# kalgeee/Uncertainty-Aware-Multimodal-Emotion-Recognition

Hardware: AMD Instinct MI355X
Metric: samples/sec fwd+bwd at B=4096 (84/256/768-dim) (higher is better)
Workload: dtype bf16; 1 GPU; configs[2]: fusion+DEER forward + MultiTaskDEERLoss + backward (dropout 0.3, gradients materialised in the flat buffer), B=4096/GPU, (B,84)+(B,256)+(B,768) bf16 feature blocks, random-init weights; optimiser step excluded as the metric defines (it maintains the packed weight copies and is timed separately); global_batch=4096, parallelism=single

## Files before the change

uncertainty-aware-multimodal-emotion-recognition_amd/csrc/chain.h:

```cpp
#pragma once
#include "common.h"
#include "nig.h"
#include "options.h"

namespace mmdeer {

constexpr int CHAIN_MAX_SEGS = 12;
constexpr int CHAIN_MAX_VECS = 16;
constexpr int CHAIN_VEC_FLOATS = 4864;

struct ChainSeg {
  const bf16_t* W;
  const float* bias;
  bf16_t* stash;
  const float* gamma;
  const float* beta;
  bf16_t* xln;
  float* out32;
  float* mean;
  float* rstd;
  int N, K, ldw;
  int kin_off, nout_off;
  int dcol_off;
  int ld_stash, nout;
// ... 15 lines not shown
  int residual;
  int res_add, res_dup;
  bf16_t* stash2;
  int stash_split;
};

struct ChainNig {
  int enabled;
  const bf16_t* e2;
  const bf16_t* w3;
  const float* evid;
  const float* targets;
  const float* stats;
  const float* gstats;
  int nblk;
  int nwp;
  bf16_t* dz2;
  float* partial_w;
  float* partial_b;
  float* loss_out;
  int* bin_counts;
  float mask_scale;
  LossCfg cfg;
};

struct ChainNigF {
  int enabled;
  const bf16_t* w3;
  const float* b3;
  int b3_stride;
  float* evid;
  float* nig_out;
  const float* targets;
  float* wstats;
};

struct ChainArgs {
  const bf16_t* X;
  int ldx, K0;
  int B;
  int ts;
  int groups;
  long long group_stride;
  int nseg;
  DropCtx drop;
  const bf16_t* aux_video; const bf16_t* aux_audio; bf16_t* aux_audio_pad;
  int aux_ldv, aux_lda;
  unsigned long long* stamps;
  ChainNig nig;
// ... 38 lines not shown
```

uncertainty-aware-multimodal-emotion-recognition_amd/csrc/chain.hip:

```cpp
#include <type_traits>
#include "gemm_kernel.inc"
#include "chain.h"
#include "options.h"
#include "nig_dev.h"
#include "ln_rows.h"

namespace mmdeer {
namespace {

template <int S>
__device__ __forceinline__ void wr_issue(const void* p) {
  static_assert(S >= 0 && S < 8, "ring slots 0..7");
  if constexpr (S == 0)
    asm volatile("global_load_dwordx4 v[248:251], %0, off\n\tglobal_load_dwordx4 v[252:255], %0, off offset:1024" ::"v"(p)
                 : "memory", "v248", "v249", "v250", "v251", "v252", "v253", "v254", "v255");
  else if constexpr (S == 1)
    asm volatile("global_load_dwordx4 v[240:243], %0, off\n\tglobal_load_dwordx4 v[244:247], %0, off offset:1024" ::"v"(p)
                 : "memory", "v240", "v241", "v242", "v243", "v244", "v245", "v246", "v247");
  else if constexpr (S == 2)
    asm volatile("global_load_dwordx4 v[232:235], %0, off\n\tglobal_load_dwordx4 v[236:239], %0, off offset:1024" ::"v"(p)
                 : "memory", "v232", "v233", "v234", "v235", "v236", "v237", "v238", "v239");
  else if constexpr (S == 3)
    asm volatile("global_load_dwordx4 v[224:227], %0, off\n\tglobal_load_dwordx4 v[228:231], %0, off offset:1024" ::"v"(p)
                 : "memory", "v224", "v225", "v226", "v227", "v228", "v229", "v230", "v231");
// ... 209 lines not shown
  f32x4 ev{0.f, 0.f, 0.f, 0.f};
  float y = 0.f;
  Nig n{0.f, 1.f, 2.f, 1.f};
  Terms t{};
  if (quad_on) {
#pragma unroll
    for (int c = 0; c < 4; ++c) load_chunk16<false>(g.w3, d * 256 + c * 64 + q * 16, w[c]);
    load_chunk16<false>(g.e2, (long long)bc * 192 + d * 64 + q * 16, x);
    ev = *reinterpret_cast<const f32x4*>(g.evid + o * 4);
    y = g.targets[o];
    n = nig_act(ev);
    t = loss_terms(n, y);
  }
  const int stat_n = g.gstats ? (int)g.gstats[3 * NIG_NSTAT] : B;
  NSTAMP(111);
  compute_finals(g.gstats ? g.gstats : g.stats, g.gstats ? 1 : g.nblk, stat_n, g.cfg, F, gs, ftmp, g.gstats ? 0 : g.nwp);
  NSTAMP(112);
  if (blockIdx.x == 0 && tid == 0) write_loss(F, g.loss_out, g.bin_counts);
  if (quad_on) {
    const f32x4 gr = loss_grad(n, t, d, stat_n, g.cfg, F);
    f32x4 dE{gr.x, gr.y * softplus_grad(ev.y), gr.z * softplus_grad(ev.z), gr.w * softplus_grad(ev.w)};
    if (!active) dE = f32x4{0.f, 0.f, 0.f, 0.f};
    float dz[16];
    float* xt = scratch + r * 195 + d * 64 + q * 16;
#pragma unroll
    for (int j = 0; j < 16; ++j) {
      xt[j] = active ? x[j] : 0.f;
      const float v = nig_dx(dE, w[0][j], w[1][j], w[2][j], w[3][j]);
      dz[j] = x[j] > 0.f ? v * g.mask_scale : 0.f;
    }
    if (active) store_chunk16<false>(g.dz2, (long long)b * 192 + d * 64 + q * 16, dz);
// ... 16 lines not shown
    for (int s = 0; s < MS; s += 2) {
      acc0 = fmaf(sde[12 * s], scratch[s * 195 + dd * 64 + j], acc0);
      acc1 = fmaf(sde[12 * s + 12], scratch[(s + 1) * 195 + dd * 64 + j], acc1);
    }
    g.partial_w[(long long)blockIdx.x * 768 + e] = acc0 + acc1;
  }
  if (tid < 12) {
    const float* sde = reinterpret_cast<const float*>(sdE) + tid;
    float bs = 0.f;
    for (int s = 0; s < MS; ++s) bs += sde[12 * s];
    g.partial_b[(long long)blockIdx.x * 12 + tid] = bs;
  }
}

template <int MS>
__device__ __forceinline__ void chain_nig_tail(const ChainNigF& g, const unsigned char* pan, int row0, int B, int tid) {
  const int wave = tid >> 6, lane = tid & 63, q = lane & 3;
  const int qw = wave - (8 - 3 * (MS / 16));
  if (qw < 0) return;
  const int d = qw % 3, blk = qw / 3;
  const int r = 16 * blk + (lane >> 2);
  const int b = row0 + r;
  const bool active = b < B;
  const int bc = active ? b : B - 1;
  float w[4][16], x[16];
#pragma unroll
  for (int c = 0; c < 4; ++c) load_chunk16<false>(g.w3, d * 256 + c * 64 + q * 16, w[c]);
  {
    const unsigned char* prow = pan + d * (MS * 128) + r * 128;
#pragma unroll
    for (int h = 0; h < 2; ++h) {
      const u32x4 raw = *reinterpret_cast<const u32x4*>(prow + (((2 * q + h) ^ (r & 7)) * 16));
      const unsigned dw[4] = {raw.x, raw.y, raw.z, raw.w};
#pragma unroll
// ... 22 lines not shown
  }
  if (g.targets) {
    const float y = g.targets[(long long)bc * 3 + d];
    const Terms t = loss_terms(n, y);
    float* slab = g.wstats + ((long long)((row0 >> 4) + blk) * 3 + d) * NIG_NSTAT;
    float v[NIG_NSTAT];
    v[0] = writer ? t.logprob : 0.f; v[1] = writer ? t.reg : 0.f; v[2] = writer ? t.kla : 0.f; v[3] = writer ? t.klb : 0.f; v[4] = writer ? t.u : 0.f;
#pragma unroll
    for (int k = 0; k < 10; ++k) {
      const bool in = writer && t.bin == k;
      v[5 + k] = in ? t.conf : 0.f; v[15 + k] = in ? t.aerr : 0.f; v[25 + k] = in ? 1.f : 0.f;
    }
#pragma unroll
    for (int i = 0; i < NIG_NSTAT; ++i) {
      const float sm = wave_sum(v[i]);
      if (lane == 0) slab[i] = sm;
    }
  }
}

template <int D, int VECF, int TS>
__device__ __forceinline__ void chain_body(const ChainKArgs& a) {
  constexpr int MS = 16 * TS, LOG_MS = TS == 1 ? 4 : 5, FLY = 2 * D;
  constexpr int G = D == 8 ? 4 : D;
  constexpr int PAN = TS == 1 ? MS * 1536 : MS * 1024;
  constexpr int AUXB = TS == 1 ? MS * 768 : 0;
  constexpr int AUX = 2 * PAN, RED = AUX + AUXB, VEC = RED + 32768, TAB = VEC + VECF * 4;
  constexpr int SEG_BYTES = (int)sizeof(ChainRecK);
  constexpr int VEC0 = CHAIN_MAX_SEGS * SEG_BYTES;
  constexpr int TAB_BYTES = VEC0 + CHAIN_MAX_VECS * (int)sizeof(ChainVecK);
  static_assert(TAB_BYTES % 16 == 0 && TAB_BYTES / 16 <= 512, "one 16-byte chunk of the tables per thread");
  static_assert(TAB + TAB_BYTES <= 160 * 1024, "LDS budget");
  __shared__ __attribute__((aligned(1024))) unsigned char lds[TAB + TAB_BYTES];
// ... 487 lines not shown
      }
      stamp(131 + 4 * si);
      if (has_ln) {
        asm volatile("s_waitcnt lgkmcnt(0)" ::: "memory");
        __builtin_amdgcn_s_barrier();
      }
      unsigned char* t = pin; pin = pout; pout = t;
      rows_in = rows_out;
    }
#pragma unroll
    for (int k = 0; k < SEG_DW; ++k) rs[k] = rn[k];
#pragma unroll
    for (int k = 0; k < 8; ++k) rl[k] = rln[k];
    stamp(5 + 3 * si);
  }
  if (a.nigf.enabled) chain_nig_tail<MS>(a.nigf, pin, row0, B, tid);
  asm volatile("s_waitcnt vmcnt(0)" ::: "memory");
}

__global__ __launch_bounds__(512) __attribute__((amdgpu_num_vgpr(112))) void chain_kernel_s16(const ChainKArgs a) {
  chain_body<4, CHAIN_VEC_FLOATS, 1>(a);
}
__global__ __launch_bounds__(512) __attribute__((amdgpu_num_vgpr(96))) void chain_kernel_s16_d8(const ChainKArgs a) {
  chain_body<8, CHAIN_VEC_FLOATS, 1>(a);
}
__global__ __launch_bounds__(512) __attribute__((amdgpu_num_vgpr(120))) void chain_kernel_s32(const ChainKArgs a) {
  chain_body<2, CHAIN_VEC_FLOATS, 2>(a);
}
__global__ __launch_bounds__(512) __attribute__((amdgpu_num_vgpr(120))) void chain_kernel_s16_d2(const ChainKArgs a) {
  chain_body<2, CHAIN_VEC_FLOATS, 1>(a);
}
// ... 114 lines not shown
    MMDEER_CHECK(ts == 1 && !a.nig.enabled && a.groups == 1, "chain: the second input panel needs 16-sample workgroups and a single-group input");
    MMDEER_CHECK(a.aux_audio && a.aux_audio_pad && ((uintptr_t)a.aux_video % 16) == 0 && a.aux_ldv % 8 == 0 && ((uintptr_t)a.aux_audio % 4) == 0 &&
                     a.aux_lda % 2 == 0 && a.aux_lda <= 128 && ((uintptr_t)a.aux_audio_pad % 16) == 0,
                 "chain: second input panel: pointers / alignment");
  }
  ChainKArgs k{};
  k.aux_video = a.aux_video; k.aux_audio = a.aux_audio; k.aux_audio_pad = a.aux_audio_pad; k.aux_ldv = a.aux_ldv; k.aux_lda = a.aux_lda;
  k.X = a.X; k.ldx = a.ldx; k.K0 = a.K0; k.B = a.B; k.groups = a.groups; k.group_stride = a.group_stride; k.drop = a.drop;
  k.stamps = a.stamps;
  k.nig = a.nig;
  k.nigf = a.nigf;
  if (a.nigf.enabled) {
    const ChainSeg& last = a.seg[a.nseg - 1];
    MMDEER_CHECK(!a.nig.enabled && last.end_layer && last.nout == 192 && !last.gamma && !last.lnb_gamma && last.fold_groups == 0,
                 "chain: the NIG tail needs a plain 192-wide last layer");
    MMDEER_CHECK(a.nigf.w3 && a.nigf.b3 && a.nigf.evid && a.nigf.nig_out && (!a.nigf.targets || a.nigf.wstats) &&
                     ((uintptr_t)a.nigf.w3 % 16) == 0 && ((uintptr_t)a.nigf.evid % 16) == 0,
                 "chain: NIG tail: NULL argument / alignment");
  }
  int vec = 0, nend = 0, nvec = 0;
  int blocks_in = a.groups * ts, width_in = a.K0, layer_first_seg = 0;
  bool layer_has_group1 = false, width_in_dup = false;
  auto add_vec = [&](const float* src, int n) { ChainVecK& v = k.vec[nvec++]; v.src = src; v.off = vec; v.n4 = n / 4; vec += n; return v.off; };
  for (int i = 0; i < a.nseg; ++i) {
    const ChainSeg& s = a.seg[i];
    MMDEER_CHECK(s.W && ((uintptr_t)s.W % 16) == 0, "chain: segment %d weights (fragment-major image) must be 16-byte aligned", i);
    MMDEER_CHECK(s.N > 0 && s.N % 64 == 0 && s.K > 0 && s.K % 64 == 0 && (s.N % 128 == 0 || s.K % 128 == 0),
                 "chain: segment %d has unsupported N = %d, K = %d", i, s.N, s.K);
    MMDEER_CHECK(!s.in_aux || a.aux_video, "chain: segment %d reads a second input panel the chain does not have", i);
    MMDEER_CHECK(s.kin_off >= 0 && s.kin_off % 64 == 0 && s.kin_off + s.K <= (s.in_aux ? 384 : width_in), "chain: segment %d reads columns [%d, %d) of a %d-wide panel", i,
                 s.kin_off, s.kin_off + s.K, s.in_aux ? 384 : width_in);
    MMDEER_CHECK(s.row_group == 0 || (s.row_group == 1 && s.fold_groups == 0 && blocks_in == ts), "chain: segment %d row group", i);
// ... 97 lines not shown
```

uncertainty-aware-multimodal-emotion-recognition_amd/csrc/common.h:

```cpp
#pragma once
#include <hip/hip_runtime.h>
#include <stdint.h>

#include <initializer_list>

namespace mmdeer {

typedef unsigned short bf16_t;
typedef __bf16 bf16x8 __attribute__((ext_vector_type(8)));
typedef float f32x4 __attribute__((ext_vector_type(4)));

__device__ __forceinline__ void store_wt4(float* p, float v) {
  asm volatile("global_store_dword %0, %1, off sc0 sc1" ::"v"(p), "v"(v) : "memory");
}
template <typename V2>
__device__ __forceinline__ void store_wt8(void* p, V2 v) {
  static_assert(sizeof(V2) == 8, "store_wt8 writes 8 bytes");
  asm volatile("global_store_dwordx2 %0, %1, off sc0 sc1" ::"v"(p), "v"(v) : "memory");
}
template <typename V4>
__device__ __forceinline__ void store_wt16(void* p, V4 v) {
  static_assert(sizeof(V4) == 16, "store_wt16 writes 16 bytes");
  asm volatile("global_store_dwordx4 %0, %1, off sc0 sc1\n\ts_nop 1" ::"v"(p), "v"(v) : "memory");
}

enum { DT_BF16 = 0, DT_F32 = 1 };

__device__ __forceinline__ float bf2f(bf16_t h) { return __uint_as_float(((unsigned)h) << 16); }
__device__ __forceinline__ bf16_t f2bf(float f) { return __builtin_bit_cast(unsigned short, (__bf16)f); }
typedef float f32x2_t __attribute__((ext_vector_type(2)));
typedef __bf16 bf16x2_t __attribute__((ext_vector_type(2)));
__device__ __forceinline__ unsigned pack_bf2(float lo, float hi) {
  return __builtin_bit_cast(unsigned, __builtin_convertvector(f32x2_t{lo, hi}, bf16x2_t));
}

template <typename T> struct Elem;
template <> struct Elem<float> {
  static constexpr int EPC = 4;
// ... 139 lines not shown
```

uncertainty-aware-multimodal-emotion-recognition_amd/csrc/gemm_tt256.hip:

```cpp
#include "gemm_kernel.inc"
#include "rowops.h"

#include <type_traits>

namespace mmdeer {
namespace {

__device__ __forceinline__ void gload16_sc1(f32x4& dst, const void* p) {
  asm volatile("global_load_dwordx4 %0, %1, off sc1" : "=v"(dst) : "v"(p) : "memory");
}
__device__ __forceinline__ void gload4_sc1(float& dst, const void* p) {
  asm volatile("global_load_dword %0, %1, off sc1" : "=v"(dst) : "v"(p) : "memory");
}

constexpr int fold_round(int want, int all) {
  int r = 1;
  while (2 * r <= want && 2 * r <= all) r *= 2;
  return r;
}

__device__ __forceinline__ void fold_tail(int tb, unsigned char* lds) {
  const __attribute__((address_space(4))) GemmFold& F =
      *(const __attribute__((address_space(4))) GemmFold*)((karg_ptr)__builtin_amdgcn_kernarg_segment_ptr() + __builtin_offsetof(GemmGroup, fold));
  const int half = threadIdx.x >> 8, b = 2 * tb + half;
  int sg = 0;
#pragma unroll
  for (int i = 1; i < GEMM_FOLD_SEGMENTS; ++i)
    if (i < F.nseg && b >= F.bstart[i]) sg = i;
// ... 344 lines not shown
```

uncertainty-aware-multimodal-emotion-recognition_amd/csrc/layout.inc:

```
X(W, ACT,  wpack,    MMDEER_FLAT_ELEMS, 0)
X(W, ACT,  wtpack,   MMDEER_FLAT_ELEMS, 0)
X(W, F32,  vpack,    MMDEER_FLAT_ELEMS, 0)
X(W, BF16, wa_pad,   INTER * AUD_PAD, 0)
X(W, BF16, wqkv_hm,  3 * FUS * FUS, 0)
X(W, F32,  wscratch, ADAM_NPART, 0)
X(W, BF16, wfpack,   MMDEER_FLAT_ELEMS, 1)
X(W, BF16, wtfpack,  MMDEER_FLAT_ELEMS, 1)
X(W, BF16, wa_frag,  INTER * AUD_PAD, 1)
X(S, BF16, audio_pad, Bz * AUD_PAD, 0)
X(S, ACT, avin, 2 * Bz * INTER, 0) X(S, ACT, avv, 2 * Bz * INTER, 0) X(S, ACT, cat, Bz * 2 * INTER, 0) X(S, ACT, y_a2, Bz * INTER, 0)
X(S, ACT, av, Bz * INTER, 0) X(S, ACT, xtok, 2 * Bz * FUS, 0) X(S, ACT, qkv, 2 * Bz * 3 * FUS, 0) X(S, ACT, obar, Bz * FUS, 0)
X(S, ACT, pool, Bz * FUS, 0) X(S, ACT, y_t3, Bz * FUS, 0) X(S, ACT, tri, Bz * FUS, 0) X(S, ACT, y_o1, Bz * FUS, 0) X(S, ACT, fused, Bz * FUS, 0)
X(S, ACT, h1, Bz * HID, 0) X(S, ACT, h2, Bz * HID, 0) X(S, ACT, e1, Bz * 3 * EV1, 0) X(S, ACT, e2, Bz * 3 * EV2, 0)
X(S, F32, probs, Bz * 8 * 4, 0) X(S, F32, evid, Bz * 12, 0)
X(S, F32, stats, 4 * nblk * 3 * NIG_NSTAT, 0)
X(S, F32, mean_a2, Bz, 0) X(S, F32, rstd_a2, Bz, 0) X(S, F32, mean_t3, Bz, 0) X(S, F32, rstd_t3, Bz, 0) X(S, F32, mean_o1, Bz, 0) X(S, F32, rstd_o1, Bz, 0)
X(S, ACT, dz2, Bz * 3 * EV2, 0) X(S, ACT, de1, Bz * 3 * EV1, 0) X(S, ACT, dh2, Bz * HID, 0) X(S, ACT, dh1, Bz * HID, 0)
X(S, ACT, dfused, Bz * FUS, 0) X(S, ACT, dz_o1, Bz * FUS, 0) X(S, ACT, dtri, Bz * FUS, 0) X(S, ACT, dz_t3, Bz * FUS, 0)
X(S, ACT, dpool, Bz * FUS, 0) X(S, ACT, dobar, Bz * FUS, 0) X(S, ACT, dqkv, 2 * Bz * 3 * FUS, 0) X(S, ACT, dxtok, 2 * Bz * FUS, 0)
X(S, ACT, dav, Bz * INTER, 0) X(S, ACT, dz_a2, Bz * INTER, 0) X(S, ACT, dcats, 2 * Bz * INTER, 0) X(S, ACT, davv, 2 * Bz * INTER, 0)
X(S, ACT, davin, 2 * Bz * INTER, 0)
X(S, F32, part_ln_o1, np * 2 * FUS, 0) X(S, F32, part_ln_t3, np * 2 * FUS, 0) X(S, F32, part_ln_a2, np * 2 * INTER, 0)
X(S, F32, part_w3, nhead * 3 * 256, 0) X(S, F32, part_b3, nhead * 3 * 4, 0)
X(S, F32, slab, SPLITK_MAX * MMDEER_FLAT_ELEMS, 0)
```

uncertainty-aware-multimodal-emotion-recognition_amd/csrc/nig.h:

```cpp
#pragma once
#include "common.h"

struct mmdeer_loss_cfg;

namespace mmdeer {

constexpr int NIG_NSTAT = 35;
constexpr int NIG_GLOBAL_STATS = 3 * NIG_NSTAT + 1;
constexpr int NIG_LOSS_OUT = 20;

struct LossCfg {
  float reg_w, kl_w, ece_w, cross_w;
  float task_w[3];
};
LossCfg loss_cfg(const mmdeer_loss_cfg& c);

constexpr int NIG_ROWS = 64;
inline int nig_nblocks(int B) { return B > 0 ? (B + NIG_ROWS - 1) / NIG_ROWS : 1; }

int launch_nig_fwd(const void* e2, const void* w3, const float* b3, int b3_stride, float* evid, float* nig_out,
                   const float* targets, float* stats, int B, int act_f32, hipStream_t s);

int launch_nig_bwd(const void* e2, const void* w3, const float* evid, const float* targets, const float* stats,
                   const float* gstats, const float* gmu, const float* gnu, const float* galpha, const float* gbeta,
                   float* devid, void* dz2, float* partial_w, float* partial_b, float* loss_out, int* bin_counts,
                   int B, int act_f32, float mask_scale, const LossCfg& cfg, int nwp, hipStream_t s);

int launch_nig_stats_sum(const float* stats, int B, float* out, int nwp, hipStream_t s);

int launch_nig_loss_stats(const float* gamma, const float* nu, const float* alpha, const float* beta,
                          const float* targets, float* stats, int B, hipStream_t s);
int launch_nig_loss_grad(const float* gamma, const float* nu, const float* alpha, const float* beta,
                         const float* targets, const float* stats, float* dgamma, float* dnu, float* dalpha,
                         float* dbeta, float* loss_out, int* bin_counts, int B, const LossCfg& cfg, hipStream_t s);

int deer_v1_nblocks(long long n);
int launch_deer_loss_v1(const float* mu, const float* nu, const float* alpha, const float* beta, const float* targets, long long n,
                        float ew, float kw, float* loss_out, float* dmu, float* dnu, float* dalpha, float* dbeta, float* partial,
                        hipStream_t s);
int launch_unc_reg_loss(const float* alpha, const float* beta, int B, int D, float dw, float sw, float* loss_out, float* dalpha,
                        float* dbeta, hipStream_t s);
// ... 11 lines not shown
```

uncertainty-aware-multimodal-emotion-recognition_amd/csrc/nig.hip:

```cpp
#include "nig.h"
#include "stamps.h"

namespace mmdeer {
namespace {
#ifdef MMDEER_STAMPS
__device__ unsigned long long g_nig_stamps[16];
#define GSTAMP(slot) MMDEER_STAMP((unsigned long long*)g_nig_stamps, slot, blockIdx.x == 0 && blockIdx.y == 0 && threadIdx.x == 0)
#endif
}
}
#include "nig_dev.h"

namespace mmdeer {
namespace {



template <bool F32>
__global__ __launch_bounds__(256) void nig_fwd_kernel(const void* e2, const void* w3, const float* b3, int b3_stride,
                                                      float* evid, float* nig_out, const float* targets, float* stats, int B) {
  const int d = blockIdx.y, tid = threadIdx.x, q = tid & 3;
  const int b = blockIdx.x * NIG_ROWS + (tid >> 2);
  const bool active = b < B;
  const int bc = active ? b : B - 1;
// ... 21 lines not shown
    nig_out[o] = n.mu; nig_out[plane + o] = n.nu; nig_out[2 * plane + o] = n.alpha; nig_out[3 * plane + o] = n.beta;
    nig_out[4 * plane + o] = alea; nig_out[5 * plane + o] = epis; nig_out[6 * plane + o] = alea + epis;
  }
  if (targets) {
    const float y = targets[(long long)bc * 3 + d];
    const Terms t = loss_terms(n, y);
    block_stats(t, writer, stats + ((long long)blockIdx.x * 3 + d) * NIG_NSTAT);
  }
}

template <bool F32>
__global__ __launch_bounds__(256) void nig_bwd_kernel(const void* e2, const void* w3, const float* evid, const float* targets,
                                                      const float* stats, const float* gstats, const float* gmu,
                                                      const float* gnu, const float* galpha, const float* gbeta, float* devid, void* dz2,
                                                      float* partial_w, float* partial_b, float* loss_out,
                                                      int* bin_counts, int B, float mask_scale, LossCfg cfg, int nwp) {
  __shared__ float gs[3][NIG_NSTAT];
  __shared__ float ftmp[NIG_FINALS_TMP];
  __shared__ f32x4 sdE[NIG_ROWS];
  __shared__ Finals F;
  __shared__ float xt[NIG_ROWS][65];
  const int d = blockIdx.y, tid = threadIdx.x, q = tid & 3, s = tid >> 2;
  const int nblk = gridDim.x;
  const int b = blockIdx.x * NIG_ROWS + s;
  const bool active = b < B;
  const int bc = active ? b : B - 1;
  const long long o = (long long)bc * 3 + d;
  GSTAMP(0);
  float w[4][16];
#pragma unroll
  for (int c = 0; c < 4; ++c) load_chunk16<F32>(w3, d * 256 + c * 64 + q * 16, w[c]);
  float x[16];
  load_chunk16<F32>(e2, (long long)bc * 192 + d * 64 + q * 16, x);
  const f32x4 ev = *reinterpret_cast<const f32x4*>(evid + o * 4);
  const bool loss_mode = targets != nullptr;
  f32x4 g{0.f, 0.f, 0.f, 0.f};
  if (loss_mode) {
    const float y = targets[o];
    GSTAMP(1);
    const int stat_n = gstats ? (int)gstats[3 * NIG_NSTAT] : B;
    compute_finals(gstats ? gstats : stats, gstats ? 1 : nblk, stat_n, cfg, F, gs, ftmp, gstats ? 0 : nwp);
    GSTAMP(2);
    if (blockIdx.x == 0 && blockIdx.y == 0 && tid == 0) write_loss(F, loss_out, bin_counts);
    const Nig n = nig_act(ev);
    const Terms t = loss_terms(n, y);
    g = loss_grad(n, t, d, stat_n, cfg, F);
    GSTAMP(3);
  } else {
    if (gmu) g.x = gmu[o];
    if (gnu) g.y = gnu[o];
    if (galpha) g.z = galpha[o];
    if (gbeta) g.w = gbeta[o];
  }
  f32x4 dE{g.x, g.y * softplus_grad(ev.y), g.z * softplus_grad(ev.z), g.w * softplus_grad(ev.w)};
  if (!active) dE = f32x4{0.f, 0.f, 0.f, 0.f};
  if (active && q == 0 && devid) *reinterpret_cast<f32x4*>(devid + o * 4) = dE;
// ... 249 lines not shown
  } else if (i == 3 * NIG_NSTAT) {
    out[i] = (float)B;
  }
}

int launch_nig_stats_sum(const float* stats, int B, float* out, int nwp, hipStream_t s) {
  MMDEER_CHECK(B > 0, "nig statistics need a non-empty batch");
  hipLaunchKernelGGL(nig_stats_sum_kernel, dim3(1), dim3(128), 0, s, stats, nig_nblocks(B), B, out, nwp);
  MMDEER_HIP(hipGetLastError());
  return 0;
}

int launch_nig_bwd(const void* e2, const void* w3, const float* evid, const float* targets, const float* stats,
                   const float* gstats, const float* gmu, const float* gnu, const float* galpha, const float* gbeta,
                   float* devid, void* dz2, float* partial_w, float* partial_b, float* loss_out, int* bin_counts,
                   int B, int act_f32, float mask_scale, const LossCfg& cfg, int nwp, hipStream_t s) {
  MMDEER_CHECK(B > 0, "nig backward needs a non-empty batch");
  dim3 grid(nig_nblocks(B), 3);
  if (act_f32)
    hipLaunchKernelGGL(nig_bwd_kernel<true>, grid, dim3(256), 0, s, e2, w3, evid, targets, stats, gstats, gmu, gnu, galpha, gbeta,
                       devid, dz2, partial_w, partial_b, loss_out, bin_counts, B, mask_scale, cfg, nwp);
  else
    hipLaunchKernelGGL(nig_bwd_kernel<false>, grid, dim3(256), 0, s, e2, w3, evid, targets, stats, gstats, gmu, gnu, galpha, gbeta,
                       devid, dz2, partial_w, partial_b, loss_out, bin_counts, B, mask_scale, cfg, nwp);
  MMDEER_HIP(hipGetLastError());
  return 0;
}

int launch_nig_loss_stats(const float* gamma, const float* nu, const float* alpha, const float* beta,
                          const float* targets, float* stats, int B, hipStream_t s) {
  MMDEER_CHECK(B > 0, "nig loss needs a non-empty batch");
  hipLaunchKernelGGL(nig_loss_stats_kernel, dim3((B + 255) / 256, 3), dim3(256), 0, s, gamma, nu, alpha, beta, targets, stats, B);
  MMDEER_HIP(hipGetLastError());
  return 0;
}

int launch_nig_loss_grad(const float* gamma, const float* nu, const float* alpha, const float* beta,
                         const float* targets, const float* stats, float* dgamma, float* dnu, float* dalpha,
                         float* dbeta, float* loss_out, int* bin_counts, int B, const LossCfg& cfg, hipStream_t s) {
// ... 52 lines not shown
```

uncertainty-aware-multimodal-emotion-recognition_amd/csrc/nig_dev.h:

```cpp
#pragma once
#include "nig.h"
#include "elem.h"

#ifndef GSTAMP
#define GSTAMP(slot) do {} while (0)
#endif

namespace mmdeer {
namespace {

typedef unsigned nig_u32x4 __attribute__((ext_vector_type(4)));

__device__ const float kEceEdges[11] = {0.0f, 0x1.99999ap-4f, 0x1.99999ap-3f, 0x1.333334p-2f, 0x1.99999ap-2f, 0x1p-1f,
                                        0x1.333334p-1f, 0x1.666666p-1f, 0x1.99999ap-1f, 0x1.ccccccp-1f, 1.0f};
constexpr float kEps = 1e-8f;
constexpr float kTwoPiEps = 6.28318530717958647692f;



struct Nig { float mu, nu, alpha, beta; };

__device__ __forceinline__ Nig nig_act(const f32x4& ev) {
#pragma clang fp contract(off)
  Nig n;
// ... 59 lines not shown
    if (lane == 0) sm[wave][i] = s;
  }
  __syncthreads();
  if (threadIdx.x < NIG_NSTAT)
    slab[threadIdx.x] = (sm[0][threadIdx.x] + sm[1][threadIdx.x]) + (sm[2][threadIdx.x] + sm[3][threadIdx.x]);
}

struct Finals {
  float sign[3][10];
  float dcross[3];
  float out[NIG_LOSS_OUT];
  int counts[3][10];
};

constexpr int NIG_FINALS_TMP = 3 * NIG_NSTAT + 30 + 3 + 3;
__device__ __forceinline__ void compute_finals(const float* stats, int nblk, int B, const LossCfg& cfg, Finals& F,
                                               float (*gs)[NIG_NSTAT], float* tmp, int nwp = 0) {
  constexpr int NV = 3 * NIG_NSTAT;
  float* const upper = tmp; float* const ece_c = tmp + NV; float* const dim_total = ece_c + 30; float* const ubar_s = dim_total + 3;
  {
    const int i = threadIdx.x & 127, h = threadIdx.x >> 7;
    float acc = 0.f;
    if (i < NV) {
      const int per = (nblk + 1) >> 1, p0 = h * per, p1 = (p0 + per < nblk) ? p0 + per : nblk;
      if (nwp == 0) {
        for (int q = p0; q < p1; q += 16) {
          float v[16];
#pragma unroll
          for (int u = 0; u < 16; ++u) {
            const int p = q + u < p1 ? q + u : p1 - 1;
            v[u] = stats[(long long)p * NV + i];
          }
#pragma unroll
          for (int u = 0; u < 16; ++u) v[u] = q + u < p1 ? v[u] : 0.f;
          acc += ((v[0] + v[1]) + (v[2] + v[3])) + ((v[4] + v[5]) + (v[6] + v[7])) +
                 (((v[8] + v[9]) + (v[10] + v[11])) + ((v[12] + v[13]) + (v[14] + v[15])));
        }
      } else {
        for (int q = p0; q < p1; q += 16) {
          float w[16][4];
#pragma unroll
          for (int u = 0; u < 16; ++u)
#pragma unroll
            for (int z = 0; z < 4; ++z) {
              const int p = q + u < p1 ? q + u : p1 - 1, wp = 4 * p + z;
              w[u][z] = stats[(long long)(wp < nwp ? wp : nwp - 1) * NV + i];
            }
          float v[16];
#pragma unroll
          for (int u = 0; u < 16; ++u) {
            const int p = q + u < p1 ? q + u : p1 - 1;
#pragma unroll
            for (int z = 0; z < 4; ++z) w[u][z] = 4 * p + z < nwp ? w[u][z] : 0.f;
            v[u] = q + u < p1 ? (w[u][0] + w[u][1]) + (w[u][2] + w[u][3]) : 0.f;
          }
          acc += ((v[0] + v[1]) + (v[2] + v[3])) + ((v[4] + v[5]) + (v[6] + v[7])) +
                 (((v[8] + v[9]) + (v[10] + v[11])) + ((v[12] + v[13]) + (v[14] + v[15])));
        }
      }
      if (h == 1) upper[i] = acc;
    }
    __syncthreads();
    if (h == 0 && i < NV) gs[i / NIG_NSTAT][i % NIG_NSTAT] = acc + upper[i];
  }
  GSTAMP(8);
  __syncthreads();
  GSTAMP(9);
  const float N = (float)B;
  if (threadIdx.x < 30) {
    const int d = threadIdx.x / 10, k = threadIdx.x - d * 10;
    const float cnt = gs[d][25 + k];
    F.counts[d][k] = (int)cnt;
    float sg = 0.f, c = 0.f;
    if (cnt > 0.f) {
      const float diff = gs[d][5 + k] / cnt - (1.0f - gs[d][15 + k] / cnt);
      c = (cnt / N) * fabsf(diff);
      sg = diff > 0.f ? 1.f : (diff < 0.f ? -1.f : 0.f);
    }
// ... 120 lines not shown
```

uncertainty-aware-multimodal-emotion-recognition_amd/csrc/stackc.hip:

```cpp
#include <cstring>

#include "../../include/mmdeer.h"
#include "../../include/mmdeer_routes.h"
#include "attention.h"
#include "common.h"
#include "gemm.h"
#include "nig.h"
#include "optim.h"
#include "options.h"
#include "chain.h"
#include "rowops.h"

namespace mmdeer {
namespace {

constexpr int TRACE_MAX = 32;
struct Trace { void** ev = nullptr; int max = 0, n = 0; const char* label[TRACE_MAX]; };
thread_local Trace g_trace;
int trace_mark(const char* label, hipStream_t s) {
  Trace& t = g_trace;
  if (!t.ev || t.n >= t.max || t.n >= TRACE_MAX) return 0;
  if (hipEventRecord((hipEvent_t)t.ev[t.n], s) != hipSuccess) { set_error("trace: hipEventRecord failed"); return -1; }
  t.label[t.n++] = label;
  return 0;
// ... 22 lines not shown
constexpr int P_AVP_W = MMDEER_P_TRIMODAL_AUDIOVISUAL_PROJECTION_WEIGHT, P_AVP_B = MMDEER_P_TRIMODAL_AUDIOVISUAL_PROJECTION_BIAS;
constexpr int P_TXT_W = MMDEER_P_TRIMODAL_TEXT_PROJECTION_WEIGHT, P_TXT_B = MMDEER_P_TRIMODAL_TEXT_PROJECTION_BIAS;
constexpr int P_TIN_W = MMDEER_P_TRIMODAL_MODALITY_ATTENTION_IN_PROJ_WEIGHT, P_TIN_B = MMDEER_P_TRIMODAL_MODALITY_ATTENTION_IN_PROJ_BIAS;
constexpr int P_TOUT_W = MMDEER_P_TRIMODAL_MODALITY_ATTENTION_OUT_PROJ_WEIGHT, P_TOUT_B = MMDEER_P_TRIMODAL_MODALITY_ATTENTION_OUT_PROJ_BIAS;
constexpr int P_TFF_W = MMDEER_P_TRIMODAL_FINAL_0_WEIGHT, P_TFF_B = MMDEER_P_TRIMODAL_FINAL_0_BIAS;
constexpr int P_TFF_G = MMDEER_P_TRIMODAL_FINAL_3_WEIGHT, P_TFF_BT = MMDEER_P_TRIMODAL_FINAL_3_BIAS;
constexpr int P_OP_W = MMDEER_P_OUTP0_WEIGHT, P_OP_B = MMDEER_P_OUTP0_BIAS, P_OP_G = MMDEER_P_OUTP3_WEIGHT, P_OP_BT = MMDEER_P_OUTP3_BIAS;
constexpr int P_FP0_W = MMDEER_P_FP0_WEIGHT, P_FP0_B = MMDEER_P_FP0_BIAS, P_FP1_W = MMDEER_P_FP3_WEIGHT, P_FP1_B = MMDEER_P_FP3_BIAS;
constexpr int P_EV0_W = MMDEER_P_HEAD0_EV0_WEIGHT, P_EV0_B = MMDEER_P_HEAD0_EV0_BIAS;
constexpr int P_EV1_W = MMDEER_P_HEAD0_EV3_WEIGHT, P_EV1_B = MMDEER_P_HEAD0_EV3_BIAS;
constexpr int P_EV2_W = MMDEER_P_HEAD0_EV6_WEIGHT, P_EV2_B = MMDEER_P_HEAD0_EV6_BIAS;

constexpr int AUD = MMDEER_AUDIO_DIM, VID = MMDEER_VIDEO_DIM, TXT = MMDEER_TEXT_DIM, INTER = MMDEER_INTER_DIM;
constexpr int FUS = MMDEER_FUSION_DIM, HID = MMDEER_HIDDEN_DIM, EV1 = 128, EV2 = 64;
constexpr int SPLITK_MAX = 8;
constexpr int AUD_PAD = 128;

struct Layout {
  using ACT = char; using BF16 = char; using F32 = float;
#define X(buf, kind, name, elems, bf16_only) kind* name;
#include "layout.inc"
#undef X
  size_t wbytes;
  size_t bytes;
};

inline size_t align_up(size_t x, size_t a = 256) { return (x + a - 1) / a * a; }

Layout make_layout(void* base, void* wbase, int B, int f32) {
  Layout L{};
// ... 565 lines not shown
  }
  if (plan.chains) {
    ChainArgs c = X.chain(n.tout.in, n.tout.K, 1, 0);
    X.fwd_seg(c, n.tout);
    X.fwd_seg(c, n.tff);
    X.fwd_seg(c, n.op);
    X.fwd_seg(c, n.fp0);
    X.fwd_seg(c, n.fp1);
    X.fwd_seg(c, n.ev0);
    X.fwd_seg(c, n.ev1);
    if (plan.nig_tail) {
      ChainNigF& g = c.nigf;
      g.enabled = 1;
      g.w3 = reinterpret_cast<const bf16_t*>(X.W(P_EV2_W)); g.b3 = X.V(P_EV2_B); g.b3_stride = 64;
      g.evid = L.evid; g.nig_out = a->nig_out; g.targets = a->targets; g.wstats = L.stats;
    }
#ifdef MMDEER_STAMPS
    c.stamps = reinterpret_cast<unsigned long long*>(L.slab);
#endif
    TRY(launch_chain(c, s));
    MARK(plan.nig_tail ? "chain F9-F18 (trimodal fusion tail + head + NIG)" : "chain F9-F17 (trimodal fusion tail + head)");
  } else {
    TRY(X.run1(X.fwd(n.tout)));
    TRY(X.run1(X.fwd(n.tff)));
    if (lnf) {
      TRY(X.fwd_ln(n.op, n.tff));
      TRY(X.fwd_ln(n.fp0, n.op));
    } else {
      TRY(X.ln_fwd(n.tff));
      TRY(X.run1(X.fwd(n.op)));
// ... 59 lines not shown
      TRY(X.run(dwg));
      MARK("weight gradients (all problems, one launch)");
      for (int i = 0; i < dwg.nprob; ++i) Exec::add_slab_segments(rt, dwg.p[i]);
    }
    if (!fold_in) {
      rt.bump = bump;
      TRY(launch_reduce_partials(rt, s));
      MARK("reduce_partials (fold)");
    }
    for (int b = first_bucket; b <= last_bucket; ++b)
      if (a->bucket_events[b]) MMDEER_HIP(hipEventRecord((hipEvent_t)a->bucket_events[b], s));
    return 0;
  };

  if (phase != 2) {
  if (!plan.nigfold)
    TRY(launch_nig_bwd(L.e2, X.W(P_EV2_W), L.evid, a->targets, L.stats, a->targets ? a->global_stats : nullptr, a->g_mu, a->g_nu, a->g_alpha, a->g_beta, nullptr,
                       L.dz2, L.part_w3, L.part_b3, a->loss_out, a->bin_counts, B, f32, X.mask_scale, cfg, plan.nwp, s));
  if (!plan.nigfold) MARK("nig_bwd (head's last layer backward + loss gradient)");
  if (plan.bchain) {
    ChainArgs c = X.chain(n.ev1.dout, n.ev1.heads * n.ev1.N, 1, 0);
    X.dx_seg(c, n.ev1);
    X.dx_seg(c, n.ev0);
    X.dx_seg(c, n.fp1);
    X.dx_seg(c, n.fp0, &n.op);
    X.dx_seg(c, n.op, &n.tff);
    X.dx_seg(c, n.tff);
    X.dx_seg(c, n.tout);
    if (plan.nigfold) {
      ChainNig& g = c.nig;
      g.enabled = 1;
      g.e2 = reinterpret_cast<const bf16_t*>(L.e2); g.w3 = reinterpret_cast<const bf16_t*>(X.W(P_EV2_W)); g.evid = L.evid;
      g.targets = a->targets; g.stats = L.stats; g.gstats = a->global_stats; g.nblk = nblk; g.nwp = plan.nwp;
      g.dz2 = reinterpret_cast<bf16_t*>(L.dz2); g.partial_w = L.part_w3; g.partial_b = L.part_b3;
      g.loss_out = a->loss_out; g.bin_counts = a->bin_counts; g.mask_scale = X.mask_scale; g.cfg = cfg;
    }
#ifdef MMDEER_STAMPS
    c.stamps = reinterpret_cast<unsigned long long*>(L.davin);
#endif
    TRY(launch_chain(c, s));
    MARK(plan.nigfold ? "chain B1-B10 (head backward + loss gradient + head / trimodal dX)" : "chain B2-B10 (head / trimodal dX)");
  } else {
    TRY(X.run1(X.dx(n.ev1)));
    TRY(X.run1(X.dx(n.ev0)));
    TRY(X.run1(X.dx(n.fp1)));
    TRY(X.run1(X.dx(n.fp0)));
  }
  if (a->g_fused) TRY(launch_add_f32(L.dfused, f32, a->g_fused, (long long)B * FUS, s));
// ... 135 lines not shown
```

uncertainty-aware-multimodal-emotion-recognition_amd/model.py:

```python
from __future__ import annotations

import ctypes as C
import math
from dataclasses import dataclass
from typing import Dict, Optional, Tuple

import torch
import torch.nn as nn

from . import _lib, synth
from .spec import DEFAULT_DIMS, DIM_NAMES, Dims, gate_param_table, param_offsets, param_table

LOSS_KEYS = ("total_loss", "nll_loss", "reg_loss", "kl_loss", "ece_loss")


@dataclass
class ModelConfig:

    audio_dim: int = 84
    video_dim: int = 256
    text_dim: int = 768
    encoder_dim: int = 256
    fusion_dim: int = 512
    emotion_dims: int = 3
# ... 187 lines not shown
        self.fusion.load_state_dict(fusion_sd)
        self.head.load_state_dict(head_sd)

    def load_numpy_state(self, state) -> None:
        sd = {k: torch.as_tensor(v) for k, v in state.items()}
        own = self.state_dict()
        for k in own:
            if k in sd:
                own[k].copy_(sd[k])

    def _workspace(self, B: int, dev: torch.device) -> torch.Tensor:
        key = (B, self.compute_f32, dev.index if dev.index is not None else 0)
        ws = self._st.workspaces.get(key)
        if ws is None:
            nbytes = _lib.load().mmdeer_workspace_bytes(B, self.compute_f32)
            ws = torch.empty(nbytes, dtype=torch.uint8, device=dev)
            self._st.workspaces[key] = ws
        return ws

    def _weights(self, dev: torch.device) -> torch.Tensor:
        key = (self.compute_f32, dev.index if dev.index is not None else 0)
        wb = self._st.weights.get(key)
        if wb is None:
            wb = torch.empty(_lib.load().mmdeer_weights_bytes(self.compute_f32), dtype=torch.uint8, device=dev)
            self._st.weights[key] = wb
            self._st.packed_key = None
        return wb

    def _param_key(self, wb: torch.Tensor):
        return (wb.data_ptr(), self._st.param_gen) + tuple((p.data_ptr(), p._version) for p in self._live)

# ... 392 lines not shown
```

Baseline: 15.67 million samples/s.

## Fold NIG loss statistics in the last forward chain workgroup via atomic ticket

The forward chain's NIG tail now takes an atomic ticket per workgroup, and the last workgroup to finish sums all per-wave statistic partials into a small global fold buffer. The backward loss-gradient code then reads this pre-folded block as if it were global stats, instead of every backward workgroup re-reducing all the per-wave partials. This removes redundant reductions from the backward critical path. In exchange it adds a grid-wide atomic, a wait on outstanding stores and cache-bypassing loads at the end of the forward pass, and requires the workspace to be zero-initialised so the counter starts at zero.

```diff
diff --git a/uncertainty-aware-multimodal-emotion-recognition_amd/csrc/chain.h b/uncertainty-aware-multimodal-emotion-recognition_amd/csrc/chain.h
--- a/uncertainty-aware-multimodal-emotion-recognition_amd/csrc/chain.h
+++ b/uncertainty-aware-multimodal-emotion-recognition_amd/csrc/chain.h
@@ -53,7 +53,6 @@
   const float* stats;
   const float* gstats;
   int nblk;
-  int nwp;
   bf16_t* dz2;
   float* partial_w;
   float* partial_b;
@@ -72,6 +71,8 @@
   float* nig_out;
   const float* targets;
   float* wstats;
+  float* fold;
+  unsigned* cnt;
 };
 
 struct ChainArgs {
diff --git a/uncertainty-aware-multimodal-emotion-recognition_amd/csrc/chain.hip b/uncertainty-aware-multimodal-emotion-recognition_amd/csrc/chain.hip
--- a/uncertainty-aware-multimodal-emotion-recognition_amd/csrc/chain.hip
+++ b/uncertainty-aware-multimodal-emotion-recognition_amd/csrc/chain.hip
@@ -247,7 +247,7 @@
   }
   const int stat_n = g.gstats ? (int)g.gstats[3 * NIG_NSTAT] : B;
   NSTAMP(111);
-  compute_finals(g.gstats ? g.gstats : g.stats, g.gstats ? 1 : g.nblk, stat_n, g.cfg, F, gs, ftmp, g.gstats ? 0 : g.nwp);
+  compute_finals(g.gstats ? g.gstats : g.stats, g.gstats ? 1 : g.nblk, stat_n, g.cfg, F, gs, ftmp);
   NSTAMP(112);
   if (blockIdx.x == 0 && tid == 0) write_loss(F, g.loss_out, g.bin_counts);
   if (quad_on) {
@@ -294,10 +294,8 @@
 }
 
 template <int MS>
-__device__ __forceinline__ void chain_nig_tail(const ChainNigF& g, const unsigned char* pan, int row0, int B, int tid) {
-  const int wave = tid >> 6, lane = tid & 63, q = lane & 3;
-  const int qw = wave - (8 - 3 * (MS / 16));
-  if (qw < 0) return;
+__device__ __forceinline__ void chain_nig_rows(const ChainNigF& g, const unsigned char* pan, int row0, int B, int qw, int lane) {
+  const int q = lane & 3;
   const int d = qw % 3, blk = qw / 3;
   const int r = 16 * blk + (lane >> 2);
   const int b = row0 + r;
@@ -350,9 +348,28 @@
 #pragma unroll
     for (int i = 0; i < NIG_NSTAT; ++i) {
       const float sm = wave_sum(v[i]);
-      if (lane == 0) slab[i] = sm;
-    }
-  }
+      if (lane == 0) store_wt4(slab + i, sm);
+    }
+  }
+}
+
+template <int MS>
+__device__ __forceinline__ void chain_nig_tail(const ChainNigF& g, const unsigned char* pan, float* scratch, int row0, int B, int tid) {
+  const int qw = (tid >> 6) - (8 - 3 * (MS / 16));
+  if (qw >= 0) chain_nig_rows<MS>(g, pan, row0, B, qw, tid & 63);
+  if (!g.targets) return;
+  asm volatile("s_waitcnt vmcnt(0)" ::: "memory");
+  __builtin_amdgcn_s_barrier();
+  volatile unsigned* ticket = reinterpret_cast<volatile unsigned*>(scratch);
+  if (tid == 0) *ticket = __hip_atomic_fetch_add(g.cnt, 1u, __ATOMIC_RELAXED, __HIP_MEMORY_SCOPE_AGENT);
+  __syncthreads();
+  if (*ticket != gridDim.x - 1) return;
+  __builtin_amdgcn_fence(__ATOMIC_ACQUIRE, "wavefront");
+  const int nwp = (B + 15) >> 4;
+  const float sum = sum_stat_partials<true, true>(g.wstats, (nwp + 3) >> 2, nwp, scratch + 16);
+  if (tid < 3 * NIG_NSTAT) g.fold[tid] = sum;
+  else if (tid == 3 * NIG_NSTAT) g.fold[tid] = (float)B;
+  if (tid == 0) __hip_atomic_store(g.cnt, 0u, __ATOMIC_RELAXED, __HIP_MEMORY_SCOPE_AGENT);
 }
 
 template <int D, int VECF, int TS>
@@ -870,7 +887,7 @@
     for (int k = 0; k < 8; ++k) rl[k] = rln[k];
     stamp(5 + 3 * si);
   }
-  if (a.nigf.enabled) chain_nig_tail<MS>(a.nigf, pin, row0, B, tid);
+  if (a.nigf.enabled) chain_nig_tail<MS>(a.nigf, pin, reinterpret_cast<float*>(pout), row0, B, tid);
   asm volatile("s_waitcnt vmcnt(0)" ::: "memory");
 }
 
@@ -1015,8 +1032,8 @@
     const ChainSeg& last = a.seg[a.nseg - 1];
     MMDEER_CHECK(!a.nig.enabled && last.end_layer && last.nout == 192 && !last.gamma && !last.lnb_gamma && last.fold_groups == 0,
                  "chain: the NIG tail needs a plain 192-wide last layer");
-    MMDEER_CHECK(a.nigf.w3 && a.nigf.b3 && a.nigf.evid && a.nigf.nig_out && (!a.nigf.targets || a.nigf.wstats) &&
-                     ((uintptr_t)a.nigf.w3 % 16) == 0 && ((uintptr_t)a.nigf.evid % 16) == 0,
+    MMDEER_CHECK(a.nigf.w3 && a.nigf.b3 && a.nigf.evid && a.nigf.nig_out && (!a.nigf.targets || (a.nigf.wstats && a.nigf.fold && a.nigf.cnt)) &&
+                     ((uintptr_t)a.nigf.w3 % 16) == 0 && ((uintptr_t)a.nigf.evid % 16) == 0 && ((uintptr_t)a.nigf.cnt % 4) == 0,
                  "chain: NIG tail: NULL argument / alignment");
   }
   int vec = 0, nend = 0, nvec = 0;
diff --git a/uncertainty-aware-multimodal-emotion-recognition_amd/csrc/common.h b/uncertainty-aware-multimodal-emotion-recognition_amd/csrc/common.h
--- a/uncertainty-aware-multimodal-emotion-recognition_amd/csrc/common.h
+++ b/uncertainty-aware-multimodal-emotion-recognition_amd/csrc/common.h
@@ -22,6 +22,12 @@
 __device__ __forceinline__ void store_wt16(void* p, V4 v) {
   static_assert(sizeof(V4) == 16, "store_wt16 writes 16 bytes");
   asm volatile("global_store_dwordx4 %0, %1, off sc0 sc1\n\ts_nop 1" ::"v"(p), "v"(v) : "memory");
+}
+__device__ __forceinline__ void gload16_sc1(f32x4& dst, const void* p) {
+  asm volatile("global_load_dwordx4 %0, %1, off sc1" : "=v"(dst) : "v"(p) : "memory");
+}
+__device__ __forceinline__ void gload4_sc1(float& dst, const void* p) {
+  asm volatile("global_load_dword %0, %1, off sc1" : "=v"(dst) : "v"(p) : "memory");
 }
 
 enum { DT_BF16 = 0, DT_F32 = 1 };
diff --git a/uncertainty-aware-multimodal-emotion-recognition_amd/csrc/gemm_tt256.hip b/uncertainty-aware-multimodal-emotion-recognition_amd/csrc/gemm_tt256.hip
--- a/uncertainty-aware-multimodal-emotion-recognition_amd/csrc/gemm_tt256.hip
+++ b/uncertainty-aware-multimodal-emotion-recognition_amd/csrc/gemm_tt256.hip
@@ -5,13 +5,6 @@
 
 namespace mmdeer {
 namespace {
-
-__device__ __forceinline__ void gload16_sc1(f32x4& dst, const void* p) {
-  asm volatile("global_load_dwordx4 %0, %1, off sc1" : "=v"(dst) : "v"(p) : "memory");
-}
-__device__ __forceinline__ void gload4_sc1(float& dst, const void* p) {
-  asm volatile("global_load_dword %0, %1, off sc1" : "=v"(dst) : "v"(p) : "memory");
-}
 
 constexpr int fold_round(int want, int all) {
   int r = 1;
diff --git a/uncertainty-aware-multimodal-emotion-recognition_amd/csrc/layout.inc b/uncertainty-aware-multimodal-emotion-recognition_amd/csrc/layout.inc
--- a/uncertainty-aware-multimodal-emotion-recognition_amd/csrc/layout.inc
+++ b/uncertainty-aware-multimodal-emotion-recognition_amd/csrc/layout.inc
@@ -22,4 +22,6 @@
 X(S, ACT, davin, 2 * Bz * INTER, 0)
 X(S, F32, part_ln_o1, np * 2 * FUS, 0) X(S, F32, part_ln_t3, np * 2 * FUS, 0) X(S, F32, part_ln_a2, np * 2 * INTER, 0)
 X(S, F32, part_w3, nhead * 3 * 256, 0) X(S, F32, part_b3, nhead * 3 * 4, 0)
-X(S, F32, slab, SPLITK_MAX * MMDEER_FLAT_ELEMS, 0)
+X(S, F32, slab, SPLITK_MAX * MMDEER_FLAT_ELEMS - NIG_FOLD_ELEMS, 0)
+X(S, F32, nig_fold, 128, 0)
+X(S, F32, nig_cnt, 64, 0)
diff --git a/uncertainty-aware-multimodal-emotion-recognition_amd/csrc/nig.h b/uncertainty-aware-multimodal-emotion-recognition_amd/csrc/nig.h
--- a/uncertainty-aware-multimodal-emotion-recognition_amd/csrc/nig.h
+++ b/uncertainty-aware-multimodal-emotion-recognition_amd/csrc/nig.h
@@ -24,7 +24,7 @@
 int launch_nig_bwd(const void* e2, const void* w3, const float* evid, const float* targets, const float* stats,
                    const float* gstats, const float* gmu, const float* gnu, const float* galpha, const float* gbeta,
                    float* devid, void* dz2, float* partial_w, float* partial_b, float* loss_out, int* bin_counts,
-                   int B, int act_f32, float mask_scale, const LossCfg& cfg, int nwp, hipStream_t s);
+                   int B, int act_f32, float mask_scale, const LossCfg& cfg, hipStream_t s);
 
 int launch_nig_stats_sum(const float* stats, int B, float* out, int nwp, hipStream_t s);
 
diff --git a/uncertainty-aware-multimodal-emotion-recognition_amd/csrc/nig.hip b/uncertainty-aware-multimodal-emotion-recognition_amd/csrc/nig.hip
--- a/uncertainty-aware-multimodal-emotion-recognition_amd/csrc/nig.hip
+++ b/uncertainty-aware-multimodal-emotion-recognition_amd/csrc/nig.hip
@@ -59,7 +59,7 @@
                                                       const float* stats, const float* gstats, const float* gmu,
                                                       const float* gnu, const float* galpha, const float* gbeta, float* devid, void* dz2,
                                                       float* partial_w, float* partial_b, float* loss_out,
-                                                      int* bin_counts, int B, float mask_scale, LossCfg cfg, int nwp) {
+                                                      int* bin_counts, int B, float mask_scale, LossCfg cfg) {
   __shared__ float gs[3][NIG_NSTAT];
   __shared__ float ftmp[NIG_FINALS_TMP];
   __shared__ f32x4 sdE[NIG_ROWS];
@@ -84,7 +84,7 @@
     const float y = targets[o];
     GSTAMP(1);
     const int stat_n = gstats ? (int)gstats[3 * NIG_NSTAT] : B;
-    compute_finals(gstats ? gstats : stats, gstats ? 1 : nblk, stat_n, cfg, F, gs, ftmp, gstats ? 0 : nwp);
+    compute_finals(gstats ? gstats : stats, gstats ? 1 : nblk, stat_n, cfg, F, gs, ftmp);
     GSTAMP(2);
     if (blockIdx.x == 0 && blockIdx.y == 0 && tid == 0) write_loss(F, loss_out, bin_counts);
     const Nig n = nig_act(ev);
@@ -364,15 +364,15 @@
 int launch_nig_bwd(const void* e2, const void* w3, const float* evid, const float* targets, const float* stats,
                    const float* gstats, const float* gmu, const float* gnu, const float* galpha, const float* gbeta,
                    float* devid, void* dz2, float* partial_w, float* partial_b, float* loss_out, int* bin_counts,
-                   int B, int act_f32, float mask_scale, const LossCfg& cfg, int nwp, hipStream_t s) {
+                   int B, int act_f32, float mask_scale, const LossCfg& cfg, hipStream_t s) {
   MMDEER_CHECK(B > 0, "nig backward needs a non-empty batch");
   dim3 grid(nig_nblocks(B), 3);
   if (act_f32)
     hipLaunchKernelGGL(nig_bwd_kernel<true>, grid, dim3(256), 0, s, e2, w3, evid, targets, stats, gstats, gmu, gnu, galpha, gbeta,
-                       devid, dz2, partial_w, partial_b, loss_out, bin_counts, B, mask_scale, cfg, nwp);
+                       devid, dz2, partial_w, partial_b, loss_out, bin_counts, B, mask_scale, cfg);
   else
     hipLaunchKernelGGL(nig_bwd_kernel<false>, grid, dim3(256), 0, s, e2, w3, evid, targets, stats, gstats, gmu, gnu, galpha, gbeta,
-                       devid, dz2, partial_w, partial_b, loss_out, bin_counts, B, mask_scale, cfg, nwp);
+                       devid, dz2, partial_w, partial_b, loss_out, bin_counts, B, mask_scale, cfg);
   MMDEER_HIP(hipGetLastError());
   return 0;
 }
diff --git a/uncertainty-aware-multimodal-emotion-recognition_amd/csrc/nig_dev.h b/uncertainty-aware-multimodal-emotion-recognition_amd/csrc/nig_dev.h
--- a/uncertainty-aware-multimodal-emotion-recognition_amd/csrc/nig_dev.h
+++ b/uncertainty-aware-multimodal-emotion-recognition_amd/csrc/nig_dev.h
@@ -97,22 +97,33 @@
 };
 
 constexpr int NIG_FINALS_TMP = 3 * NIG_NSTAT + 30 + 3 + 3;
-__device__ __forceinline__ void compute_finals(const float* stats, int nblk, int B, const LossCfg& cfg, Finals& F,
-                                               float (*gs)[NIG_NSTAT], float* tmp, int nwp = 0) {
+
+template <bool WAVE, bool SC1>
+__device__ __forceinline__ float sum_stat_partials(const float* stats, int nblk, int nwp, float* upper) {
   constexpr int NV = 3 * NIG_NSTAT;
-  float* const upper = tmp; float* const ece_c = tmp + NV; float* const dim_total = ece_c + 30; float* const ubar_s = dim_total + 3;
+  auto ld = [](const float* p) __attribute__((always_inline)) {
+    float v;
+    if constexpr (SC1) gload4_sc1(v, p);
+    else v = *p;
+    return v;
+  };
   {
     const int i = threadIdx.x & 127, h = threadIdx.x >> 7;
     float acc = 0.f;
     if (i < NV) {
       const int per = (nblk + 1) >> 1, p0 = h * per, p1 = (p0 + per < nblk) ? p0 + per : nblk;
-      if (nwp == 0) {
+      if constexpr (!WAVE) {
         for (int q = p0; q < p1; q += 16) {
           float v[16];
 #pragma unroll
           for (int u = 0; u < 16; ++u) {
             const int p = q + u < p1 ? q + u : p1 - 1;
-            v[u] = stats[(long long)p * NV + i];
+            v[u] = ld(stats + (long long)p * NV + i);
+          }
+          if constexpr (SC1) {
+            asm volatile("s_waitcnt vmcnt(0)" ::: "memory");
+#pragma unroll
+            for (int u = 0; u < 16; ++u) asm volatile("" : "+v"(v[u]));
           }
 #pragma unroll
           for (int u = 0; u < 16; ++u) v[u] = q + u < p1 ? v[u] : 0.f;
@@ -127,8 +138,15 @@
 #pragma unroll
             for (int z = 0; z < 4; ++z) {
               const int p = q + u < p1 ? q + u : p1 - 1, wp = 4 * p + z;
-              w[u][z] = stats[(long long)(wp < nwp ? wp : nwp - 1) * NV + i];
+              w[u][z] = ld(stats + (long long)(wp < nwp ? wp : nwp - 1) * NV + i);
             }
+          if constexpr (SC1) {
+            asm volatile("s_waitcnt vmcnt(0)" ::: "memory");
+#pragma unroll
+            for (int u = 0; u < 16; ++u)
+#pragma unroll
+              for (int z = 0; z < 4; ++z) asm volatile("" : "+v"(w[u][z]));
+          }
           float v[16];
 #pragma unroll
           for (int u = 0; u < 16; ++u) {
@@ -144,7 +162,17 @@
       if (h == 1) upper[i] = acc;
     }
     __syncthreads();
-    if (h == 0 && i < NV) gs[i / NIG_NSTAT][i % NIG_NSTAT] = acc + upper[i];
+    return h == 0 && i < NV ? acc + upper[i] : 0.f;
+  }
+}
+
+__device__ __forceinline__ void compute_finals(const float* stats, int nblk, int B, const LossCfg& cfg, Finals& F,
+                                               float (*gs)[NIG_NSTAT], float* tmp) {
+  constexpr int NV = 3 * NIG_NSTAT;
+  float* const upper = tmp; float* const ece_c = tmp + NV; float* const dim_total = ece_c + 30; float* const ubar_s = dim_total + 3;
+  {
+    const float sum = sum_stat_partials<false, false>(stats, nblk, 0, upper);
+    if (threadIdx.x < NV) gs[threadIdx.x / NIG_NSTAT][threadIdx.x % NIG_NSTAT] = sum;
   }
   GSTAMP(8);
   __syncthreads();
diff --git a/uncertainty-aware-multimodal-emotion-recognition_amd/csrc/stackc.hip b/uncertainty-aware-multimodal-emotion-recognition_amd/csrc/stackc.hip
--- a/uncertainty-aware-multimodal-emotion-recognition_amd/csrc/stackc.hip
+++ b/uncertainty-aware-multimodal-emotion-recognition_amd/csrc/stackc.hip
@@ -60,6 +60,9 @@
 constexpr int AUD = MMDEER_AUDIO_DIM, VID = MMDEER_VIDEO_DIM, TXT = MMDEER_TEXT_DIM, INTER = MMDEER_INTER_DIM;
 constexpr int FUS = MMDEER_FUSION_DIM, HID = MMDEER_HIDDEN_DIM, EV1 = 128, EV2 = 64;
 constexpr int SPLITK_MAX = 8;
+constexpr int NIG_FOLD_ELEMS = 128 + 64;
+static_assert(kParams[P_EV2_B].off + NIG_FOLD_ELEMS == MMDEER_FLAT_ELEMS && MMDEER_NUM_PARAMS == P_EV2_B + 3, "the slab's tail is the head's last-layer biases");
+static_assert(NIG_GLOBAL_STATS <= 128 && (SPLITK_MAX * (size_t)MMDEER_FLAT_ELEMS * 4) % 256 == 0, "nig_fold holds the folded block; the fields tile the old slab");
 constexpr int AUD_PAD = 128;
 
 struct Layout {
@@ -655,6 +658,7 @@
       g.enabled = 1;
       g.w3 = reinterpret_cast<const bf16_t*>(X.W(P_EV2_W)); g.b3 = X.V(P_EV2_B); g.b3_stride = 64;
       g.evid = L.evid; g.nig_out = a->nig_out; g.targets = a->targets; g.wstats = L.stats;
+      g.fold = L.nig_fold; g.cnt = reinterpret_cast<unsigned*>(L.nig_cnt);
     }
 #ifdef MMDEER_STAMPS
     c.stamps = reinterpret_cast<unsigned long long*>(L.slab);
@@ -744,9 +748,10 @@
   };
 
   if (phase != 2) {
+  const float* const gstats = a->global_stats ? a->global_stats : plan.nig_tail ? L.nig_fold : nullptr;
   if (!plan.nigfold)
-    TRY(launch_nig_bwd(L.e2, X.W(P_EV2_W), L.evid, a->targets, L.stats, a->targets ? a->global_stats : nullptr, a->g_mu, a->g_nu, a->g_alpha, a->g_beta, nullptr,
-                       L.dz2, L.part_w3, L.part_b3, a->loss_out, a->bin_counts, B, f32, X.mask_scale, cfg, plan.nwp, s));
+    TRY(launch_nig_bwd(L.e2, X.W(P_EV2_W), L.evid, a->targets, L.stats, a->targets ? gstats : nullptr, a->g_mu, a->g_nu, a->g_alpha, a->g_beta, nullptr,
+                       L.dz2, L.part_w3, L.part_b3, a->loss_out, a->bin_counts, B, f32, X.mask_scale, cfg, s));
   if (!plan.nigfold) MARK("nig_bwd (head's last layer backward + loss gradient)");
   if (plan.bchain) {
     ChainArgs c = X.chain(n.ev1.dout, n.ev1.heads * n.ev1.N, 1, 0);
@@ -761,7 +766,7 @@
       ChainNig& g = c.nig;
       g.enabled = 1;
       g.e2 = reinterpret_cast<const bf16_t*>(L.e2); g.w3 = reinterpret_cast<const bf16_t*>(X.W(P_EV2_W)); g.evid = L.evid;
-      g.targets = a->targets; g.stats = L.stats; g.gstats = a->global_stats; g.nblk = nblk; g.nwp = plan.nwp;
+      g.targets = a->targets; g.stats = L.stats; g.gstats = gstats; g.nblk = nblk;
       g.dz2 = reinterpret_cast<bf16_t*>(L.dz2); g.partial_w = L.part_w3; g.partial_b = L.part_b3;
       g.loss_out = a->loss_out; g.bin_counts = a->bin_counts; g.mask_scale = X.mask_scale; g.cfg = cfg;
     }
diff --git a/uncertainty-aware-multimodal-emotion-recognition_amd/model.py b/uncertainty-aware-multimodal-emotion-recognition_amd/model.py
--- a/uncertainty-aware-multimodal-emotion-recognition_amd/model.py
+++ b/uncertainty-aware-multimodal-emotion-recognition_amd/model.py
@@ -225,7 +225,7 @@
         ws = self._st.workspaces.get(key)
         if ws is None:
             nbytes = _lib.load().mmdeer_workspace_bytes(B, self.compute_f32)
-            ws = torch.empty(nbytes, dtype=torch.uint8, device=dev)
+            ws = torch.zeros(nbytes, dtype=torch.uint8, device=dev)
             self._st.workspaces[key] = ws
         return ws
 
```

Result: no change. 15.57 million samples/s (-0.6%).
